# shg8/3DGS.cpp

Measured on AMD Instinct MI355X. Metric: frames/sec at 1920×1080, 1M Gaussians, higher is better.
Workload: dtype f32

## Files before the change

3dgs.cpp_amd/csrc/gs_bin_l2.hip:

```cpp
#include "gs_bin.h"

namespace gs {

struct SlabDesc {
    uint32_t off, c_total;
    uint32_t kmin;
    int32_t sh;
    uint32_t b_lo, b_hi;
    uint32_t ready;
    uint32_t pad;
    uint32_t cur[64];
};
static_assert(sizeof(SlabDesc) == 288, "descriptor layout");

struct BuildArgs {
    BinGrid g;
    uint32_t* cand;
    const uint32_t* bin_count;
    const float* depth;
    const ushort4* aabb;
    uint32_t* ranges;
    uint32_t* sorted_gid;
    Counters* counters;
    uint32_t capacity;
    uint32_t cand_capacity;
    SlabDesc* slabs;
    uint32_t slab_capacity;
    uint32_t epoch;
    uint64_t* stamps;
    const uint32_t* l1_words;
    uint32_t l1_cap;
};

__device__ __forceinline__ uint32_t bin_candidates(const BuildArgs& a, uint32_t bin) {
    return a.l1_words ? a.l1_words[(size_t)(kL1FusedCursor0 + bin) * kL1FusedStride] : a.bin_count[bin];
}
__device__ __forceinline__ uint32_t bin_offset(const BuildArgs& a, uint32_t bin) {
    return a.l1_words ? ((bin >> a.g.grid_shift) * a.g.bins_x + (bin & ((1u << a.g.grid_shift) - 1u))) * a.l1_cap : a.bin_count[kBinOffsets + bin];
}
__device__ __forceinline__ void bin_close_one_pass(const BuildArgs& a, uint32_t& c, int tid) {
    if (!a.l1_words) return;
    if (tid == 0 && c != 0) {
        atomicAdd(&a.counters->bin_entries, c);
        atomicMax(&a.counters->max_bin, c);
    }
    if (c > a.l1_cap) {
        if (tid == 0) atomicOr(&a.counters->overflow, 1u);
        c = 0;
    }
}
__device__ __forceinline__ void one_pass_visible(const BuildArgs& a) {
    if (!a.l1_words || blockIdx.x != 0 || threadIdx.x >= kVisRegions) return;
    uint32_t v = a.l1_words[(size_t)threadIdx.x * kL1FusedStride];
    for (int o = WAVE / 2; o != 0; o >>= 1) v += (uint32_t)__shfl_xor((int)v, o);
    if ((threadIdx.x & (WAVE - 1)) == 0 && v != 0) atomicAdd(&a.counters->visible, v);
}

__device__ __forceinline__ uint32_t bin_local_box(const BinGrid& g, uint32_t bin, ushort4 box) {
    const int S = 1 << g.bin_shift;
    const int ox = (int)(bin & ((1u << g.grid_shift) - 1u)) << g.bin_shift, oy = (int)(bin >> g.grid_shift) << g.bin_shift;
    const int lx0 = max((int)box.x, ox) - ox, ly0 = max((int)box.y, oy) - oy;
    const int lx1 = min((int)box.z, ox + S) - ox, ly1 = min((int)box.w, oy + S) - oy;
    return (uint32_t)lx0 | ((uint32_t)ly0 << 8) | ((uint32_t)lx1 << 16) | ((uint32_t)ly1 << 24);
}

constexpr int kBuildSlots = 16;

#ifdef GS_BUILD_TIMING
__device__ unsigned long long g_build_t[1024][10];
#define BUILD_ROW(v) uint32_t build_row = (v)
#define BUILD_ROW_SET(v) build_row = (v)
#define BUILD_T(i) do { if (threadIdx.x == 0) g_build_t[build_row][i] = wall_clock64(); } while (0)
#else
#define BUILD_ROW(v) do { } while (0)
#define BUILD_ROW_SET(v) do { } while (0)
#define BUILD_T(i) do { } while (0)
#endif

template <int R2, int THREADS, bool SORT>
struct BuildLayout {
    static constexpr int NW = THREADS / WAVE;
    static constexpr int MAXC = SORT ? THREADS * 16 : 0;
    static constexpr int SS = 64 * R2;
    static constexpr bool CACHE_BOX = SORT && R2 <= 4;
    static constexpr int TABLES = 3 * SS + kBuildSlots * SS / 2 + (SORT ? 0 : kBuildSlots * WAVE);
    static constexpr int WCNT = SORT ? NW * 256 : 0;
    static constexpr int T_OFF = (SORT && (CACHE_BOX || TABLES > MAXC)) ? 2 * MAXC : 0;
    static constexpr int WORDS = (T_OFF + TABLES > 2 * MAXC + WCNT) ? T_OFF + TABLES : 2 * MAXC + WCNT;
};

template <int R2, int THREADS, bool SORT>
__global__ __launch_bounds__(THREADS) void k_bin_build(BuildArgs a) {
    frame_stamp(a.stamps, ST_L2);
    one_pass_visible(a);
    BUILD_ROW(blockIdx.x);
    using L = BuildLayout<R2, THREADS, SORT>;
    constexpr int NW = L::NW, MAXC = L::MAXC, SS = L::SS, PER = kBuildSlots / NW;
    extern __shared__ uint32_t smem[];
    uint32_t* const s_key = smem;
    uint32_t* const s_id = smem + MAXC;
    uint32_t (*const s_wcnt)[256] = reinterpret_cast<uint32_t(*)[256]>(smem + 2 * MAXC);
    uint32_t* const t_cnt = smem + L::T_OFF;
    uint32_t* const t_cur = t_cnt + SS;
    uint16_t (*const r_cnt)[SS] = reinterpret_cast<uint16_t(*)[SS]>(t_cnt + 3 * SS);
    uint32_t* const w_ids = t_cnt + 3 * SS + kBuildSlots * SS / 2;
    __shared__ uint32_t scratch[NW];
    __shared__ uint32_t s_seg;

    const int tid = threadIdx.x, lane = tid & (WAVE - 1), w = tid / WAVE;
    const uint32_t bin = ((blockIdx.x / a.g.bins_x) << a.g.grid_shift) | (blockIdx.x % a.g.bins_x);
    BUILD_T(0);
    uint32_t c, off;
    c = bin_candidates(a, bin);
    off = bin_offset(a, bin);
    bin_close_one_pass(a, c, tid);
    if ((uint64_t)off + c > a.cand_capacity) c = 0;
    if (SORT && c > (uint32_t)MAXC) {
        if (tid == 0) atomicOr(&a.counters->overflow, 2u);
        c = 0;
    }
    BUILD_T(1);
    if (SORT && c != 0) {
        constexpr int kRounds = 16;
        {
            uint32_t g[kRounds], k[kRounds];
#pragma unroll
            for (int r = 0; r < kRounds; ++r) {
                const uint32_t e = r * THREADS + tid;
                g[r] = e < c ? a.cand[off + e] : 0u;
            }
#pragma unroll
            for (int r = 0; r < kRounds; ++r) {
                const uint32_t e = r * THREADS + tid;
                k[r] = e < c ? __float_as_uint(a.depth[g[r]]) : 0u;
            }
#pragma unroll
            for (int r = 0; r < kRounds; ++r) {
                const uint32_t e = r * THREADS + tid;
                if (e < c) {
                    s_id[e] = g[r];
                    s_key[e] = k[r];
                }
            }
        }
        BUILD_T(2);
        const uint64_t lt_mask = (1ull << lane) - 1ull;
        const int rounds = (int)((c + THREADS - 1) / THREADS);
        const uint32_t wbase = (uint32_t)w * (uint32_t)rounds * WAVE;
#pragma unroll 1
        for (int pass = 0; pass < 4; ++pass) {
            const int shift = pass * 8;
            for (int k = tid; k < NW * 256; k += THREADS) s_wcnt[k >> 8][k & 255] = 0;
            __syncthreads();
            uint32_t key[kRounds], id[kRounds], rank[kRounds];
#pragma unroll
            for (int r = 0; r < kRounds; ++r) {
                key[r] = 0;
                id[r] = 0;
                rank[r] = 0;
                if (r < rounds) {
                    const uint32_t e = wbase + r * WAVE + lane;
                    const bool ok = e < c;
                    if (ok) {
                        key[r] = s_key[e];
                        id[r] = s_id[e];
                    }
                    const uint32_t d = (key[r] >> shift) & 255u;
                    const uint64_t okm = __ballot(ok);
                    uint32_t mlo = (uint32_t)okm, mhi = (uint32_t)(okm >> 32);
#pragma unroll
                    for (int bit = 0; bit < 8; ++bit) {
                        const uint32_t mine = (d >> bit) & 1u;
                        const uint64_t b = __builtin_amdgcn_ballot_w64(mine != 0);
                        const uint32_t splat = 0u - mine;
                        mlo &= ~((uint32_t)b ^ splat);
                        mhi &= ~((uint32_t)(b >> 32) ^ splat);
                    }
                    const uint64_t m = ((uint64_t)mhi << 32) | mlo;
                    uint32_t old = 0;
                    const int leader = m ? (__ffsll((unsigned long long)m) - 1) : 0;
                    if (ok && lane == leader) {
                        old = s_wcnt[w][d];
                        s_wcnt[w][d] = old + (uint32_t)__popcll(m);
                    }
                    old = __shfl(old, leader, WAVE);
                    rank[r] = old + (uint32_t)__popcll(m & lt_mask);
                }
            }
            __syncthreads();
            {
                uint32_t cw[NW], cnt = 0;
                if (tid < 256) {
#pragma unroll
                    for (int k = 0; k < NW; ++k) {
                        cw[k] = s_wcnt[k][tid];
                        cnt += cw[k];
                    }
                }
                uint32_t all;
                uint32_t excl = block_excl_scan<THREADS>(cnt, scratch, &all);
                if (tid < 256) {
#pragma unroll
                    for (int k = 0; k < NW; ++k) {
                        s_wcnt[k][tid] = excl;
                        excl += cw[k];
                    }
                }
            }
            __syncthreads();
#pragma unroll
            for (int r = 0; r < kRounds; ++r) {
                if (r < rounds) {
                    const uint32_t e = wbase + r * WAVE + lane;
                    if (e < c) {
                        const uint32_t d = (key[r] >> shift) & 255u;
                        const uint32_t pos = s_wcnt[w][d] + rank[r];
                        s_key[pos] = key[r];
                        s_id[pos] = id[r];
                    }
                }
            }
            __syncthreads();
        }
        BUILD_T(3);
        if (L::CACHE_BOX) {
            ushort4 box[kRounds];
#pragma unroll
            for (int r = 0; r < kRounds; ++r) {
                const uint32_t e = r * THREADS + tid;
                box[r] = e < c ? a.aabb[s_id[e]] : make_ushort4(0, 0, 0, 0);
            }
#pragma unroll
            for (int r = 0; r < kRounds; ++r) {
                const uint32_t e = r * THREADS + tid;
                if (e < c) s_key[e] = bin_local_box(a.g, bin, box[r]);
            }
        }
    }
    BUILD_T(4);
    for (int t = tid; t < SS; t += THREADS) t_cnt[t] = 0;
    __syncthreads();
    const uint32_t nch = (c + WAVE - 1) / WAVE;
    auto chunk_columns = [&](uint32_t ch, uint64_t (&col)[R2], uint32_t& gid) {
        const uint32_t e = ch * WAVE + lane;
        uint32_t box = 0;
        gid = 0;
        if (e < c) {
            gid = SORT ? s_id[e] : a.cand[off + e];
            box = L::CACHE_BOX ? s_key[e] : bin_local_box(a.g, bin, a.aabb[gid]);
        }
        packed_cover_masks<R2>(a.g.bin_shift, box, col);
#pragma unroll
        for (int r = 0; r < R2; ++r)
            col[r] = (R2 == 1 || __builtin_amdgcn_ballot_w64(col[r] != 0) != 0) ? wave_transpose64(col[r], lane) : 0ull;
    };
    {
        uint32_t acc[R2];
#pragma unroll
        for (int r = 0; r < R2; ++r) acc[r] = 0;
        for (uint32_t ch = w; ch < nch; ch += NW) {
            uint64_t col[R2];
            uint32_t gid;
            chunk_columns(ch, col, gid);
#pragma unroll
            for (int r = 0; r < R2; ++r) acc[r] += (uint32_t)__popcll(col[r]);
        }
#pragma unroll
        for (int r = 0; r < R2; ++r)
            if (acc[r]) atomicAdd(&t_cnt[r * 64 + lane], acc[r]);
    }
    __syncthreads();
    BUILD_T(5);
    {
        uint32_t v[(SS + THREADS - 1) / THREADS], sum = 0;
#pragma unroll
        for (int k = 0; k < (SS + THREADS - 1) / THREADS; ++k) {
            const int t = tid * ((SS + THREADS - 1) / THREADS) + k;
            v[k] = t < SS ? t_cnt[t] : 0u;
            sum += v[k];
        }
        uint32_t d_bin;
        uint32_t excl = block_excl_scan<THREADS>(sum, scratch, &d_bin);
        if (tid == 0) {
            const uint32_t seg = d_bin ? atomicAdd(&a.counters->instances, d_bin) : 0u;
            s_seg = seg;
            if ((uint64_t)seg + d_bin > a.capacity) atomicOr(&a.counters->overflow, 1u);
        }
        __syncthreads();
        const uint32_t S = 1u << a.g.bin_shift;
        const uint32_t ox = (bin & ((1u << a.g.grid_shift) - 1u)) << a.g.bin_shift, oy = (bin >> a.g.grid_shift) << a.g.bin_shift;
#pragma unroll
        for (int k = 0; k < (SS + THREADS - 1) / THREADS; ++k) {
            const int t = tid * ((SS + THREADS - 1) / THREADS) + k;
            if (t < SS) {
                const uint32_t lx = (uint32_t)t & (S - 1), ly = (uint32_t)t >> a.g.bin_shift;
                const uint32_t x = ox + lx, y = oy + ly;
                const uint64_t start64 = (uint64_t)s_seg + excl;
                const uint32_t start = start64 > a.capacity ? a.capacity : (uint32_t)start64;
                const uint32_t end = start64 + v[k] > a.capacity ? a.capacity : (uint32_t)(start64 + v[k]);
                if (ly < S && x < a.g.tiles_x && y < a.g.tiles_y) {
                    a.ranges[2 * (y * a.g.tiles_x + x)] = v[k] ? start : 0u;
                    a.ranges[2 * (y * a.g.tiles_x + x) + 1] = v[k] ? end : 0u;
                }
                t_cur[t] = start;
            }
            excl += v[k];
        }
    }
    __syncthreads();
    BUILD_T(6);
    const __amdgpu_buffer_rsrc_t out = __builtin_amdgcn_make_buffer_rsrc(a.sorted_gid, 0, a.capacity * 4u, 0x27000);
    int par = 0;
    for (uint32_t rb = 0; rb < nch; rb += kBuildSlots, par ^= 1) {
        uint64_t col[PER][R2];
#pragma unroll
        for (int j = 0; j < PER; ++j) {
            const int slot = w * PER + j;
            uint32_t gid;
            chunk_columns(rb + slot, col[j], gid);
#pragma unroll
            for (int r = 0; r < R2; ++r) r_cnt[slot][r * 64 + lane] = (uint16_t)__popcll(col[j][r]);
            if (!SORT) w_ids[slot * WAVE + lane] = gid;
        }
        __syncthreads();
        for (int t = tid; t < SS; t += THREADS) {
            uint32_t run = 0;
#pragma unroll
            for (int k = 0; k < kBuildSlots; ++k) {
                const uint32_t v = r_cnt[k][t];
                r_cnt[k][t] = (uint16_t)run;
                run += v;
            }
            t_cur[(par ^ 1) * SS + t] = t_cur[par * SS + t] + run;
        }
        __syncthreads();
#pragma unroll
        for (int j = 0; j < PER; ++j) {
            const int slot = w * PER + j;
            const uint32_t ch = rb + slot;
            const uint32_t* ids = SORT ? s_id + (ch < nch ? ch : 0u) * WAVE : w_ids + slot * WAVE;
#pragma unroll
            for (int r = 0; r < R2; ++r) {
                if (__builtin_amdgcn_ballot_w64(col[j][r] != 0) == 0) continue;
                walk_column(col[j][r], t_cur[par * SS + r * 64 + lane] + r_cnt[slot][r * 64 + lane], out, ids);
            }
        }
    }
    BUILD_T(7);
}

#ifdef GS_BUILD_TIMING
extern "C" int gs_debug_build_timing(unsigned long long* out ) {
    return hipMemcpyFromSymbol(out, HIP_SYMBOL(g_build_t), sizeof(unsigned long long) * 1024 * 10) == hipSuccess ? 0 : -1;
}
#endif

__device__ __forceinline__ __amdgpu_buffer_rsrc_t uniform_rsrc(const void* p, uint32_t bytes) {
    const uint64_t addr = reinterpret_cast<uint64_t>(p);
    const uint32_t lo = (uint32_t)__builtin_amdgcn_readfirstlane((int)(uint32_t)addr);
    const uint32_t hi = (uint32_t)__builtin_amdgcn_readfirstlane((int)(uint32_t)(addr >> 32));
    return __builtin_amdgcn_make_buffer_rsrc(reinterpret_cast<void*>(((uint64_t)hi << 32) | lo), 0,
                                             __builtin_amdgcn_readfirstlane((int)bytes), 0x27000);
}

__device__ __forceinline__ uint32_t cover16(uint32_t pb) {
    const uint32_t lx0 = pb & 15u, ly0 = (pb >> 4) & 15u, lx1 = (pb >> 8) & 15u, ly1 = (pb >> 12) & 15u;
    const uint32_t xm = ((2u << lx1) - (1u << lx0)) & 15u;
    const uint32_t rows = (16u << (4u * ly1)) - (1u << (4u * ly0));
    return (xm * 0x1111u) & rows;
}

template <int ROUNDS>
struct FastLayout {
    static constexpr int THREADS = 1024, NW = THREADS / WAVE, MAXC = THREADS * ROUNDS;
    static constexpr int WCNT_WORDS = NW * 512 / 2;
    static constexpr int MISC_WORDS = 64 + 64 + NW * 64;
    static constexpr int TAIL = WCNT_WORDS > MISC_WORDS ? WCNT_WORDS : MISC_WORDS;
    static constexpr int WORDS = 2 * MAXC + TAIL;
};

template <int ROUNDS, int MODE = 0>
__device__ __forceinline__ void bin_fast_body(const BuildArgs& a) {
    constexpr bool SLABS = MODE != 0;
    using L = FastLayout<ROUNDS>;
    constexpr int THREADS = L::THREADS, NW = L::NW, MAXC = L::MAXC;
    extern __shared__ uint32_t smem[];
    uint32_t* const s_pay = smem;
    uint32_t* const s_key = smem + MAXC;
    uint16_t (*const s_wcnt)[512] = reinterpret_cast<uint16_t(*)[512]>(smem + 2 * MAXC);
    uint32_t* const s_id = smem + MAXC;
    uint16_t* const s_box = reinterpret_cast<uint16_t*>(smem);
    uint16_t (*const s_tbl)[64] = reinterpret_cast<uint16_t(*)[64]>(smem + MAXC / 2);
    uint32_t* const t_cnt = smem + 2 * MAXC;
    uint32_t* const t_cur = t_cnt + 64;
    uint32_t (*const s_seg)[64] = reinterpret_cast<uint32_t(*)[64]>(t_cnt + 128);
    __shared__ uint32_t scratch[NW], scratch_hi[NW];
    __shared__ uint32_t s_seg0, s_flag;
    constexpr int kSlotBits = SLABS ? 16 : 14;
    constexpr uint32_t kSlotMask = (1u << kSlotBits) - 1u;
    constexpr uint32_t kMaxInBin = SLABS ? 65535u : (uint32_t)MAXC;
    constexpr int kMaxSlabs = 16;
    __shared__ uint32_t g_cur[SLABS ? 64 : 1], t_tot[SLABS ? 64 : 1];
    __shared__ uint32_t slab_first[SLABS ? kMaxSlabs + 1 : 1];
    __shared__ uint32_t cnt2[(MODE == 1 || MODE == 3) ? kMaxSlabs : 1][64];
    __shared__ uint32_t s_fill;
    __shared__ uint16_t q_order[MODE == 3 ? 1024 : 1];
    __shared__ uint32_t q_item, q_planned;

    BUILD_ROW(MODE == 2 ? 1023u : blockIdx.x);
    if constexpr (MODE != 2) frame_stamp(a.stamps, ST_L2);
    if constexpr (MODE != 2) one_pass_visible(a);
    int tid = threadIdx.x, lane = tid & (WAVE - 1), w = tid / WAVE;
    auto screen_bin = [&](uint32_t i) { return ((i / a.g.bins_x) << a.g.grid_shift) | (i % a.g.bins_x); };
    uint32_t bin = screen_bin(MODE == 3 ? 0u : blockIdx.x);
    bool slab_item = MODE == 2;
    BUILD_T(0);
    uint32_t c_total = 0, off = 0;
    auto bin_extent = [&]() {
        c_total = (uint32_t)__builtin_amdgcn_readfirstlane((int)bin_candidates(a, bin));
        off = (uint32_t)__builtin_amdgcn_readfirstlane((int)bin_offset(a, bin));
        bin_close_one_pass(a, c_total, tid);
        if ((uint64_t)off + c_total > a.cand_capacity) c_total = 0;
        if (c_total > kMaxInBin) {
            if (tid == 0) atomicOr(&a.counters->overflow, 2u);
            c_total = 0;
        }
    };
    if constexpr (MODE == 0 || MODE == 1) bin_extent();
    if (tid == 0) s_flag = 0;
    BUILD_T(1);
#define multi (MODE == 2 ? true : (MODE == 1 ? c_total > (uint32_t)MAXC : (MODE == 3 ? (slab_item || c_total > (uint32_t)MAXC) : false)))
    uint32_t c = multi ? 0u : c_total;
    int rounds = (int)((c + THREADS - 1) / THREADS);
    typedef uint32_t u32x3 __attribute__((ext_vector_type(3)));
#define recs uniform_rsrc(a.cand + (size_t)kCandWords * off, c_total * 12u)
    uint64_t lt_mask = (1ull << lane) - 1ull;
    uint32_t wbase = (uint32_t)w * (uint32_t)rounds * WAVE;
    auto refresh = [&]() {
        int t = threadIdx.x;
        asm volatile("" : "+v"(t));
        tid = t;
        lane = t & (WAVE - 1);
        w = t / WAVE;
        lt_mask = (1ull << lane) - 1ull;
        wbase = (uint32_t)w * (uint32_t)rounds * WAVE;
    };
    auto radix_pass = [&](int shift, int db, uint32_t sub) {
        const uint32_t dmask = (1u << db) - 1u;
        for (int k = tid; k < NW * 512 / 2; k += THREADS) reinterpret_cast<uint32_t*>(&s_wcnt[0][0])[k] = 0;
        __syncthreads();
        uint32_t key[ROUNDS], pay[ROUNDS], rank[ROUNDS];
#pragma unroll
        for (int r = 0; r < ROUNDS; ++r) {
            key[r] = 0;
            pay[r] = 0;
            rank[r] = 0;
            if (r < rounds) {
                const uint32_t e = wbase + r * WAVE + lane;
                const bool ok = e < c;
                if (ok) {
                    key[r] = s_key[e] - sub;
                    pay[r] = s_pay[e];
                }
                const uint32_t d = (key[r] >> shift) & dmask;
                const uint64_t okm = __ballot(ok);
                uint32_t mlo = (uint32_t)okm, mhi = (uint32_t)(okm >> 32);
#pragma unroll
                for (int bit = 0; bit < 9; ++bit) {
                    if (bit < db) {
                        const uint32_t mine = (d >> bit) & 1u;
                        const uint64_t b = __builtin_amdgcn_ballot_w64(mine != 0);
                        const uint32_t splat = 0u - mine;
                        mlo &= ~((uint32_t)b ^ splat);
                        mhi &= ~((uint32_t)(b >> 32) ^ splat);
                    }
                }
                const uint64_t m = ((uint64_t)mhi << 32) | mlo;
                uint32_t old = 0;
                const int leader = m ? (__ffsll((unsigned long long)m) - 1) : 0;
                if (ok && lane == leader) {
                    old = s_wcnt[w][d];
                    s_wcnt[w][d] = (uint16_t)(old + (uint32_t)__popcll(m));
                }
                old = __shfl(old, leader, WAVE);
                rank[r] = old + (uint32_t)__popcll(m & lt_mask);
            }
        }
        __syncthreads();
        {
            uint32_t cw[NW], cnt = 0;
            if (tid < 512) {
#pragma unroll
                for (int k = 0; k < NW; ++k) {
                    cw[k] = s_wcnt[k][tid];
                    cnt += cw[k];
                }
            }
            uint32_t all;
            uint32_t excl = block_excl_scan<THREADS>(cnt, scratch, &all);
            if (tid < 512) {
#pragma unroll
                for (int k = 0; k < NW; ++k) {
                    s_wcnt[k][tid] = (uint16_t)excl;
                    excl += cw[k];
                }
            }
        }
        __syncthreads();
#pragma unroll
        for (int r = 0; r < ROUNDS; ++r) {
            if (r < rounds) {
                const uint32_t e = wbase + r * WAVE + lane;
                if (e < c) {
                    const uint32_t d = (key[r] >> shift) & dmask;
                    const uint32_t pos = (uint32_t)s_wcnt[w][d] + rank[r];
                    s_key[pos] = key[r];
                    s_pay[pos] = pay[r];
                }
            }
        }
        __syncthreads();
    };
    auto block_minmax = [&](uint32_t lo, uint32_t hi, uint32_t& kmin, uint32_t& span) {
#pragma unroll
        for (int d = 1; d < WAVE; d <<= 1) {
            lo = min(lo, (uint32_t)__shfl_xor((int)lo, d, WAVE));
            hi = max(hi, (uint32_t)__shfl_xor((int)hi, d, WAVE));
        }
        __syncthreads();
        if (lane == 0) {
            scratch[w] = lo;
            scratch_hi[w] = hi;
        }
        __syncthreads();
#pragma unroll
        for (int k = 0; k < NW; ++k) {
            lo = min(lo, scratch[k]);
            hi = max(hi, scratch_hi[k]);
        }
        kmin = (uint32_t)__builtin_amdgcn_readfirstlane((int)lo);
        span = (uint32_t)__builtin_amdgcn_readfirstlane((int)hi) - kmin;
    };
    auto key_range = [&](uint32_t& kmin, uint32_t& span) {
        uint32_t lo = 0xFFFFFFFFu, hi = 0u;
#pragma unroll
        for (int r = 0; r < ROUNDS; ++r) {
            const uint32_t e = r * THREADS + tid;
            if (r < rounds && e < c) {
                const uint32_t k = s_key[e];
                lo = min(lo, k);
                hi = max(hi, k);
            }
        }
        block_minmax(lo, hi, kmin, span);
    };
    auto sort_by_key_lsd = [&](uint32_t kmin, uint32_t span) {
        const int bits = span ? 32 - __builtin_clz(span) : 0;
        const int npass = (bits + 8) / 9;
        const int db = npass ? (bits + npass - 1) / npass : 0;
#pragma unroll 1
        for (int pass = 0; pass < npass; ++pass) radix_pass(pass * db, db, pass == 0 ? kmin : 0u);
        return npass ? kmin : 0u;
    };
    constexpr uint32_t kMsdBuckets = 4096, kMsdBucketMax = 64;
    uint32_t* const m_cnt = smem + 2 * MAXC;
    uint16_t* const m_start = reinterpret_cast<uint16_t*>(smem + 2 * MAXC + kMsdBuckets / 2);
    static_assert(kMsdBuckets * 4 <= L::TAIL * 4, "the bucket tables live in the counters' area");
    auto sort_by_key_msd = [&](uint32_t kmin, uint32_t span) -> bool {
        const int bits = 32 - __builtin_clz(span);
        const int sh = bits > 12 ? bits - 12 : 0;
        for (uint32_t k = tid; k < kMsdBuckets / 2; k += THREADS) m_cnt[k] = 0;
        __syncthreads();
        uint32_t key[ROUNDS], pay[ROUNDS];
#pragma unroll
        for (int r = 0; r < ROUNDS; ++r) {
            const uint32_t e = r * THREADS + tid;
            key[r] = 0;
            pay[r] = 0;
            if (r < rounds && e < c) {
                key[r] = s_key[e];
                pay[r] = s_pay[e];
                const uint32_t b = (key[r] - kmin) >> sh;
                atomicAdd(&m_cnt[b >> 1], 1u << (16u * (b & 1u)));
            }
        }
        __syncthreads();
        {
            const uint2 w2 = reinterpret_cast<const uint2*>(m_cnt)[tid];
            const uint32_t v0 = w2.x & 0xFFFFu, v1 = w2.x >> 16, v2 = w2.y & 0xFFFFu, v3 = w2.y >> 16;
            uint32_t all;
            uint32_t excl = block_excl_scan<THREADS>(v0 + v1 + v2 + v3, scratch, &all);
            if (max(max(v0, v1), max(v2, v3)) > kMsdBucketMax) s_flag = 2;
            reinterpret_cast<uint2*>(m_cnt)[tid] = make_uint2(0u, 0u);
            ushort4 st;
            st.x = (unsigned short)excl;
            st.y = (unsigned short)(excl + v0);
            st.z = (unsigned short)(excl + v0 + v1);
            st.w = (unsigned short)(excl + v0 + v1 + v2);
            reinterpret_cast<ushort4*>(m_start)[tid] = st;
        }
        __syncthreads();
        if (__builtin_amdgcn_readfirstlane((int)s_flag) == 2) {
            __syncthreads();
            if (tid == 0) s_flag = 0;
            return false;
        }
#pragma unroll
        for (int r = 0; r < ROUNDS; ++r) {
            const uint32_t e = r * THREADS + tid;
            if (r < rounds && e < c) {
                const uint32_t b = (key[r] - kmin) >> sh;
                const uint32_t old = atomicAdd(&m_cnt[b >> 1], 1u << (16u * (b & 1u)));
                const uint32_t pos = (uint32_t)m_start[b] + ((old >> (16u * (b & 1u))) & 0xFFFFu);
                s_key[pos] = key[r];
                s_pay[pos] = pay[r];
            }
        }
        __syncthreads();
        uint32_t dst[ROUNDS];
#pragma unroll
        for (int r = 0; r < ROUNDS; ++r) {
            const uint32_t e = r * THREADS + tid;
            dst[r] = 0xFFFFFFFFu;
            if (r < rounds && e < c) {
                const uint32_t k = s_key[e];
                pay[r] = s_pay[e];
                key[r] = k;
                const uint32_t b = (k - kmin) >> sh;
                const uint32_t j0 = m_start[b], j1 = b + 1 < kMsdBuckets ? (uint32_t)m_start[b + 1] : c;
                uint32_t before = 0;
                for (uint32_t j = j0; j < j1; ++j) {
                    const uint32_t kj = s_key[j];
                    before += (kj < k || (kj == k && j < e)) ? 1u : 0u;
                }
                dst[r] = j0 + before;
            }
        }
        __syncthreads();
#pragma unroll
        for (int r = 0; r < ROUNDS; ++r)
            if (dst[r] != 0xFFFFFFFFu) {
                s_key[dst[r]] = key[r];
                s_pay[dst[r]] = pay[r];
            }
        __syncthreads();
        return true;
    };
    auto sort_by_key = [&](bool try_msd) -> uint32_t {
        uint32_t kmin, span;
        key_range(kmin, span);
        if (span == 0) return 0u;
        if constexpr (ROUNDS <= 12) {
            if (try_msd && sort_by_key_msd(kmin, span)) return 0u;
        }
        return sort_by_key_lsd(kmin, span);
    };
    const int S = 1 << a.g.bin_shift;
    auto place_lists = [&](uint32_t v, uint32_t* cursors) {
        uint32_t d_bin;
        const uint32_t excl = block_excl_scan<THREADS>(v, scratch, &d_bin);
        if (tid == 0) {
            const uint32_t seg = d_bin ? atomicAdd(&a.counters->instances, d_bin) : 0u;
            s_seg0 = seg;
            if ((uint64_t)seg + d_bin > a.capacity) atomicOr(&a.counters->overflow, 1u);
        }
        __syncthreads();
        if (tid < 64) {
            const uint32_t ox = (bin & ((1u << a.g.grid_shift) - 1u)) << a.g.bin_shift, oy = (bin >> a.g.grid_shift) << a.g.bin_shift;
            const uint32_t lx = (uint32_t)tid & (uint32_t)(S - 1), ly = (uint32_t)tid >> a.g.bin_shift;
            const uint32_t x = ox + lx, y = oy + ly;
            const uint64_t start64 = (uint64_t)s_seg0 + excl;
            const uint32_t start = start64 > a.capacity ? a.capacity : (uint32_t)start64;
            const uint32_t end = start64 + v > a.capacity ? a.capacity : (uint32_t)(start64 + v);
            if (ly < (uint32_t)S && x < a.g.tiles_x && y < a.g.tiles_y) {
                a.ranges[2 * (y * a.g.tiles_x + x)] = v ? start : 0u;
                a.ranges[2 * (y * a.g.tiles_x + x) + 1] = v ? end : 0u;
            }
            cursors[tid] = start;
        }
    };
    uint32_t n_slabs = 1, g_kmin = 0;
    int g_sh = 0;
    auto plan_bin = [&]() {
    if constexpr (MODE == 1 || MODE == 3) if (!slab_item && multi) {
        uint32_t lo = 0xFFFFFFFFu, hi = 0u;
        for (uint32_t base = 0; base < c_total; base += 8 * THREADS) {
            uint32_t k[8];
#pragma unroll
            for (int r = 0; r < 8; ++r) k[r] = __builtin_amdgcn_raw_buffer_load_b32(recs, (base + r * THREADS + tid) * 12u, 0, 0);
#pragma unroll
            for (int r = 0; r < 8; ++r)
                if (base + r * THREADS + tid < c_total) {
                    lo = min(lo, k[r]);
                    hi = max(hi, k[r]);
                }
        }
        uint32_t span;
        block_minmax(lo, hi, g_kmin, span);
        const int bits = span ? 32 - __builtin_clz(span) : 0;
        g_sh = bits > 12 ? bits - 12 : 0;
        for (uint32_t k = tid; k < kMsdBuckets / 2; k += THREADS) m_cnt[k] = 0;
        for (uint32_t k = tid; k < (uint32_t)kMaxSlabs * 64u; k += THREADS) cnt2[k >> 6][k & 63u] = 0;
        __syncthreads();
        for (uint32_t base = 0; base < c_total; base += 8 * THREADS) {
            uint32_t k[8];
#pragma unroll
            for (int r = 0; r < 8; ++r) k[r] = __builtin_amdgcn_raw_buffer_load_b32(recs, (base + r * THREADS + tid) * 12u, 0, 0);
#pragma unroll
            for (int r = 0; r < 8; ++r)
                if (base + r * THREADS + tid < c_total) {
                    const uint32_t bk = (k[r] - g_kmin) >> g_sh;
                    atomicAdd(&m_cnt[bk >> 1], 1u << (16u * (bk & 1u)));
                }
        }
        __syncthreads();
        {
            const uint2 w2 = reinterpret_cast<const uint2*>(m_cnt)[tid];
            const uint32_t v0 = w2.x & 0xFFFFu, v1 = w2.x >> 16, v2 = w2.y & 0xFFFFu, v3 = w2.y >> 16;
            uint32_t all;
            const uint32_t excl = block_excl_scan<THREADS>(v0 + v1 + v2 + v3, scratch, &all);
            if (max(max(v0, v1), max(v2, v3)) > (uint32_t)MAXC) s_flag = 3;
            ushort4 st;
            st.x = (unsigned short)excl;
            st.y = (unsigned short)(excl + v0);
            st.z = (unsigned short)(excl + v0 + v1);
            st.w = (unsigned short)(excl + v0 + v1 + v2);
            reinterpret_cast<ushort4*>(m_start)[tid] = st;
            if (tid == 0) {
                slab_first[0] = 0;
                s_fill = 1;
            }
        }
        __syncthreads();
        for (int k = 0; k < kMaxSlabs; ++k) {
            const uint32_t base = m_start[slab_first[k]];
            if (c_total - base <= (uint32_t)MAXC) break;
#pragma unroll
            for (int j = 0; j < 4; ++j) {
                const uint32_t bk = 4u * tid + j;
                const uint32_t p0 = m_start[bk], p1 = bk + 1 < kMsdBuckets ? (uint32_t)m_start[bk + 1] : c_total;
                if (p0 - base <= (uint32_t)MAXC && p1 - base > (uint32_t)MAXC && bk > slab_first[k]) {
                    slab_first[k + 1] = bk;
                    s_fill = k + 2;
                }
            }
            __syncthreads();
            if (s_fill != (uint32_t)k + 2) {
                if (tid == 0) s_flag = 3;
                break;
            }
        }
        __syncthreads();
        n_slabs = (uint32_t)__builtin_amdgcn_readfirstlane((int)s_fill);
        if (tid == 0) slab_first[n_slabs] = kMsdBuckets;
        const uint32_t remaining = c_total - m_start[slab_first[n_slabs - 1]];
        if (__builtin_amdgcn_readfirstlane((int)s_flag) == 3 || remaining > (uint32_t)MAXC) {
            if (tid == 0) atomicOr(&a.counters->overflow, 2u);
            n_slabs = 0;
        }
        __syncthreads();
        if (tid == 0) s_flag = 0;
        for (uint32_t base = 0; n_slabs != 0 && base < c_total; base += 8 * THREADS) {
            uint32_t k[8], bx[8];
#pragma unroll
            for (int r = 0; r < 8; ++r) {
                const u32x3 rec = __builtin_amdgcn_raw_buffer_load_b96(recs, (base + r * THREADS + tid) * 12u, 0, 0);
                k[r] = rec.x;
                bx[r] = rec.z;
            }
#pragma unroll
            for (int r = 0; r < 8; ++r) {
                const bool valid = base + r * THREADS + tid < c_total;
                const uint32_t bk = (k[r] - g_kmin) >> g_sh;
                uint32_t sl = 0;
                for (uint32_t j = 1; j < n_slabs; ++j) sl += bk >= slab_first[j] ? 1u : 0u;
                const uint32_t pb = bx[r];
                if (S == 4) {
                    const uint32_t cm = valid ? cover16(pb) : 0u;
                    if (__builtin_amdgcn_ballot_w64(cm != 0) == 0) continue;
                    uint64_t bal[16];
#pragma unroll
                    for (int t = 0; t < 16; ++t) bal[t] = __builtin_amdgcn_ballot_w64(((cm >> t) & 1u) != 0);
                    for (uint32_t j = 0; j < n_slabs; ++j) {
                        const uint64_t mk = __builtin_amdgcn_ballot_w64(valid && sl == j);
                        if (mk == 0) continue;
                        uint32_t mine = 0;
#pragma unroll
                        for (int t = 0; t < 16; ++t) mine = lane == t ? (uint32_t)__popcll(bal[t] & mk) : mine;
                        if (lane < 16 && mine != 0) atomicAdd(&cnt2[j][lane], mine);
                    }
                } else if (valid) {
                    const uint32_t lx0 = pb & 15u, ly0 = (pb >> 4) & 15u, lx1 = (pb >> 8) & 15u, ly1 = (pb >> 12) & 15u;
                    for (uint32_t y = ly0; y <= ly1; ++y)
                        for (uint32_t x = lx0; x <= lx1; ++x) atomicAdd(&cnt2[sl][(y << a.g.bin_shift) + x], 1u);
                }
            }
        }
        __syncthreads();
        if (tid < 64) {
            uint32_t run = 0;
            for (uint32_t k = 0; k < n_slabs; ++k) {
                const uint32_t v = cnt2[k][tid];
                cnt2[k][tid] = run;
                run += v;
            }
            t_tot[tid] = run;
        }
        __syncthreads();
        place_lists(tid < 64 ? t_tot[tid] : 0u, g_cur);
        __syncthreads();
        if (tid == 0) {
            const uint32_t base = n_slabs ? atomicAdd(&a.counters->slabs, n_slabs) : 0u;
            s_seg0 = base;
            if (base + n_slabs > a.slab_capacity) atomicOr(&a.counters->overflow, 2u);
        }
        __syncthreads();
        const uint32_t dbase = (uint32_t)__builtin_amdgcn_readfirstlane((int)s_seg0);
        if (dbase + n_slabs <= a.slab_capacity) {
            auto put = [&](uint32_t* p, uint32_t v) {
                if constexpr (MODE == 3) __hip_atomic_store(p, v, __ATOMIC_RELAXED, __HIP_MEMORY_SCOPE_AGENT);
                else *p = v;
            };
            for (uint32_t k = 0; k < n_slabs; ++k) {
                SlabDesc* d = a.slabs + dbase + k;
                if (tid < 64) put(&d->cur[tid], g_cur[tid] + cnt2[k][tid]);
                if (tid == 64) {
                    put(&d->off, off);
                    put(&d->c_total, c_total);
                    put(&d->kmin, g_kmin);
                    put(reinterpret_cast<uint32_t*>(&d->sh), (uint32_t)g_sh);
                    put(&d->b_lo, slab_first[k]);
                    put(&d->b_hi, slab_first[k + 1]);
                }
            }
            if constexpr (MODE == 3) {
                asm volatile("s_waitcnt vmcnt(0)" ::: "memory");
                __syncthreads();
                if (tid == 0) {
                    for (uint32_t k = 0; k < n_slabs; ++k)
                        __hip_atomic_store(&a.slabs[dbase + k].ready, a.epoch, __ATOMIC_RELAXED, __HIP_MEMORY_SCOPE_AGENT);
                    asm volatile("s_waitcnt vmcnt(0)" ::: "memory");
                }
            }
        }
        n_slabs = 0;
    }
    };
    if constexpr (MODE == 1) plan_bin();
    auto slab_body = [&](const uint32_t slab) {
    if constexpr (SLABS) if (multi) {
        const uint32_t b_lo = slab_first[slab], b_hi = slab_first[slab + 1];
        __syncthreads();
        if (tid == 0) s_fill = 0;
        __syncthreads();
        for (uint32_t base = 0; base < c_total; base += 8 * THREADS) {
            uint32_t k[8], bx[8];
#pragma unroll
            for (int r = 0; r < 8; ++r) {
                const u32x3 rec = __builtin_amdgcn_raw_buffer_load_b96(recs, (base + r * THREADS + tid) * 12u, 0, 0);
                k[r] = rec.x;
                bx[r] = rec.z;
            }
#pragma unroll
            for (int r = 0; r < 8; ++r) {
                const uint32_t e = base + r * THREADS + tid;
                const uint32_t bk = (k[r] - g_kmin) >> g_sh;
                const bool mine = e < c_total && bk >= b_lo && bk < b_hi;
                const uint64_t mm = __builtin_amdgcn_ballot_w64(mine);
                if (mm != 0) {
                    uint32_t at = 0;
                    if (lane == __ffsll((unsigned long long)mm) - 1) at = atomicAdd(&s_fill, (uint32_t)__popcll(mm));
                    at = (uint32_t)__builtin_amdgcn_readlane((int)at, __ffsll((unsigned long long)mm) - 1) + (uint32_t)__popcll(mm & lt_mask);
                    if (mine && at < (uint32_t)MAXC) {
                        s_key[at] = k[r];
                        s_pay[at] = e | (bx[r] << kSlotBits);
                    }
                }
            }
        }
        __syncthreads();
        c = min((uint32_t)__builtin_amdgcn_readfirstlane((int)s_fill), (uint32_t)MAXC);
        rounds = (int)((c + THREADS - 1) / THREADS);
        wbase = (uint32_t)w * (uint32_t)rounds * WAVE;
    }
    for (int attempt = 0; c != 0 && attempt < 2; ++attempt) {
        uint32_t tid12 = (uint32_t)tid * 12u;
        asm volatile("" : "+v"(tid12));
        constexpr int HR = ROUNDS <= 8 ? ROUNDS : ROUNDS / 2;
        const int h_end = multi ? 0 : ROUNDS;
#pragma unroll
        for (int h = 0; h < h_end; h += HR) {
            uint32_t k[HR], b[HR];
#pragma unroll
            for (int r = 0; r < HR; ++r) {
                k[r] = 0;
                b[r] = 0;
                if (h + r < rounds) {
                    const u32x3 rec = __builtin_amdgcn_raw_buffer_load_b96(recs, tid12 + (uint32_t)(h + r) * (THREADS * 12u), 0, 0);
                    k[r] = rec.x;
                    b[r] = rec.z;
                }
            }
#pragma unroll
            for (int r = 0; r < HR; ++r) {
                const uint32_t e = (h + r) * THREADS + tid;
                if (h + r < rounds && e < c) {
                    s_key[e] = k[r];
                    s_pay[e] = e | (b[r] << kSlotBits);
                }
            }
        }
        if (attempt == 0) BUILD_T(2);
        sort_by_key(attempt == 0);
        if (attempt == 0) BUILD_T(8);
        refresh();
        uint32_t my_id[ROUNDS], run_len[(ROUNDS + 3) / 4];
        bool too_long = false;
#pragma unroll
        for (int q = 0; q < (ROUNDS + 3) / 4; ++q) run_len[q] = 0;
#pragma unroll
        for (int r = 0; r < ROUNDS; ++r) {
            const uint32_t e = r * THREADS + tid;
            my_id[r] = 0;
            if (r < rounds && e < c) {
                my_id[r] = __builtin_amdgcn_raw_buffer_load_b32(recs, (s_pay[e] & kSlotMask) * 12u + 4u, 0, 0);
                const uint32_t k = s_key[e];
                if (attempt == 0 && (e == 0 || s_key[e - 1] != k) && e + 1 < c && s_key[e + 1] == k) {
                    uint32_t more = 1;
                    while (e + more + 1 < c && more < 64 && s_key[e + more + 1] == k) ++more;
                    if (e + more + 1 < c && s_key[e + more + 1] == k) too_long = true;
                    run_len[r / 4] |= more << (8 * (r % 4));
                }
            }
        }
        if (too_long) s_flag = 1;
        __syncthreads();
        const bool redo = __builtin_amdgcn_readfirstlane((int)s_flag) != 0;
#pragma unroll
        for (int r = 0; r < ROUNDS; ++r) {
            const uint32_t e = r * THREADS + tid;
            if (r < rounds && e < c) s_id[e] = my_id[r];
        }
        __syncthreads();
        if (attempt == 0) BUILD_T(9);
        if (multi && redo) {
            if (tid == 0) atomicOr(&a.counters->overflow, 2u);
            __syncthreads();
            if (tid == 0) s_flag = 0;
            break;
        }
        if (!redo) {
#pragma unroll
            for (int r = 0; r < ROUNDS; ++r) {
                const uint32_t more = (run_len[r / 4] >> (8 * (r % 4))) & 255u;
                if (more != 0) {
                    const uint32_t e = r * THREADS + tid;
                    for (uint32_t i = e + 1; i <= e + more; ++i) {
                        const uint32_t vi = s_id[i], vp = s_pay[i];
                        uint32_t j = i;
                        while (j > e && s_id[j - 1] > vi) {
                            s_id[j] = s_id[j - 1];
                            s_pay[j] = s_pay[j - 1];
                            --j;
                        }
                        s_id[j] = vi;
                        s_pay[j] = vp;
                    }
                }
            }
            __syncthreads();
            break;
        }
        const uint32_t id_base = sort_by_key(false);
        uint32_t nk[ROUNDS], ni[ROUNDS], nb[ROUNDS];
#pragma unroll
        for (int r = 0; r < ROUNDS; ++r) {
            const uint32_t e = r * THREADS + tid;
            nk[r] = ni[r] = nb[r] = 0;
            if (r < rounds && e < c) {
                const uint32_t pw = s_pay[e];
                nk[r] = __builtin_amdgcn_raw_buffer_load_b32(recs, (pw & kSlotMask) * 12u, 0, 0);
                ni[r] = s_id[e] + id_base;
                nb[r] = pw >> kSlotBits;
            }
        }
        __syncthreads();
#pragma unroll
        for (int r = 0; r < ROUNDS; ++r) {
            const uint32_t e = r * THREADS + tid;
            if (r < rounds && e < c) {
                u32x3 rec = {nk[r], ni[r], nb[r]};
                __builtin_amdgcn_raw_buffer_store_b96(rec, recs, e * 12u, 0, 0);
            }
        }
        __threadfence_block();
        if (tid == 0) s_flag = 0;
        __syncthreads();
    }
#undef recs
    BUILD_T(3);
    refresh();
    const uint32_t nch = (c + WAVE - 1) / WAVE;
    {
        uint32_t pb16[ROUNDS];
#pragma unroll
        for (int r = 0; r < ROUNDS; ++r) {
            const uint32_t e = r * THREADS + tid;
            pb16[r] = e < c ? s_pay[e] >> kSlotBits : 0u;
        }
        __syncthreads();
        for (uint32_t k = tid; k < (uint32_t)MAXC / 2; k += THREADS) smem[MAXC / 2 + k] = 0;
        if (tid < 64) t_cnt[tid] = 0;
        __syncthreads();
#pragma unroll
        for (int r = 0; r < ROUNDS; ++r) {
            const uint32_t e = r * THREADS + tid;
            const uint32_t pb = pb16[r];
            if (e < c) s_box[e] = (uint16_t)pb;
            if (S == 4) {
                const uint32_t ch = (uint32_t)r * NW + (uint32_t)__builtin_amdgcn_readfirstlane(w);
                if (ch < nch) {
                    const uint32_t cm = e < c ? cover16(pb) : 0u;
                    uint32_t mine = 0;
#pragma unroll
                    for (int t = 0; t < 16; ++t) {
                        const uint64_t bal = __builtin_amdgcn_ballot_w64(((cm >> t) & 1u) != 0);
                        mine = lane == t ? (uint32_t)__popcll(bal) : mine;
                    }
                    s_tbl[ch][lane] = (uint16_t)mine;
                }
            }
        }
        if (S != 4) {
            __syncthreads();
            for (uint32_t ch = w; ch < nch; ch += NW) {
                const uint32_t e = ch * WAVE + lane;
                const uint32_t pb = e < c ? (uint32_t)s_box[e] : 0xFFFFu;
                uint64_t m[1];
                cover_masks<1>(3, (int)(pb & 15u), (int)((pb >> 4) & 15u), (int)((pb >> 8) & 15u) + 1, (int)(pb >> 12) + 1, m);
                if (e >= c) m[0] = 0;
                s_tbl[ch][lane] = (uint16_t)__popcll(wave_transpose64(m[0], lane));
            }
        }
    }
    __syncthreads();
    BUILD_T(4);
    {
        const int t = tid & 63, g = tid >> 6;
        const uint32_t per = (nch + NW - 1) / NW;
        const uint32_t q0 = min(nch, (uint32_t)g * per), q1 = min(nch, q0 + per);
        uint32_t sum = 0;
        for (uint32_t q = q0; q < q1; ++q) sum += s_tbl[q][t];
        s_seg[g][t] = sum;
        __syncthreads();
        if (tid < 64) {
            uint32_t run = 0;
#pragma unroll
            for (int k = 0; k < NW; ++k) {
                const uint32_t v = s_seg[k][tid];
                s_seg[k][tid] = run;
                run += v;
            }
            t_cnt[tid] = run;
        }
        __syncthreads();
        uint32_t run = s_seg[g][t];
        for (uint32_t q = q0; q < q1; ++q) {
            const uint32_t v = s_tbl[q][t];
            s_tbl[q][t] = (uint16_t)run;
            run += v;
        }
    }
    __syncthreads();
    BUILD_T(5);
    if (!multi) {
        place_lists(tid < 64 ? t_cnt[tid] : 0u, t_cur);
    } else if (tid < 64) {
        t_cur[tid] = g_cur[tid];
    }
    __syncthreads();
    BUILD_T(6);
    refresh();
    const __amdgpu_buffer_rsrc_t out = __builtin_amdgcn_make_buffer_rsrc(a.sorted_gid, 0, a.capacity * 4u, 0x27000);
    for (uint32_t ch = w; ch < nch; ch += NW) {
        const uint32_t e = ch * WAVE + lane;
        const bool valid = e < c;
        const uint32_t id = valid ? s_id[e] : 0u;
        const uint32_t pb = valid ? (uint32_t)s_box[e] : 0u;
        const int lx0 = (int)(pb & 15u), ly0 = (int)((pb >> 4) & 15u), lx1 = (int)((pb >> 8) & 15u), ly1 = (int)(pb >> 12);
        const uint32_t base = t_cur[lane] + (uint32_t)s_tbl[ch][lane];
        if (S == 4) {
            const uint32_t cm = valid ? cover16(pb) : 0u;
#pragma unroll
            for (int t = 0; t < 16; ++t) {
                const bool covered = ((cm >> t) & 1u) != 0;
                const uint64_t bal = __builtin_amdgcn_ballot_w64(covered);
                if (bal == 0) continue;
                const uint32_t rank = __builtin_amdgcn_mbcnt_hi((uint32_t)(bal >> 32), __builtin_amdgcn_mbcnt_lo((uint32_t)bal, 0u));
                const uint32_t pos = (uint32_t)__builtin_amdgcn_readlane((int)base, t) + rank;
                __builtin_amdgcn_raw_buffer_store_b32(id, out, covered ? pos * 4u : 0xFFFFFFFFu, 0, 0);
            }
        } else {
            uint64_t m[1];
            cover_masks<1>(3, lx0, ly0, lx1 + 1, ly1 + 1, m);
            if (!valid) m[0] = 0;
            walk_column(wave_transpose64(m[0], lane), base, out, s_id + ch * WAVE);
        }
    }
    if (multi && tid < 64) g_cur[tid] += t_cnt[tid];
    };
    if constexpr (MODE == 0) {
        slab_body(0u);
    } else if constexpr (MODE == 1) {
        if (n_slabs != 0) slab_body(0u);
    } else if constexpr (MODE == 3) {
        const uint32_t n_bins = a.g.bins_x * a.g.bins_y;
        {
            uint32_t* const cnt = smem;
            const uint32_t mine = (uint32_t)tid < n_bins ? bin_candidates(a, screen_bin((uint32_t)tid)) : 0u;
            cnt[tid] = mine;
            if (tid == 0) q_planned = 0;
            __syncthreads();
            if (mine > (uint32_t)MAXC) atomicAdd(&q_planned, 1u);
            if ((uint32_t)tid < n_bins) {
                uint32_t before = 0;
                for (uint32_t j = 0; j < n_bins; ++j) {
                    const uint32_t v = cnt[j];
                    before += (v > mine || (v == mine && j < (uint32_t)tid)) ? 1u : 0u;
                }
                q_order[before] = (uint16_t)tid;
            }
            __syncthreads();
        }
        const uint32_t n_planned = (uint32_t)__builtin_amdgcn_readfirstlane((int)q_planned);
        for (;;) {
            __syncthreads();
            refresh();
            if (tid == 0) {
                q_item = atomicAdd(&a.counters->q_head, 1u);
                s_flag = 0;
            }
            __syncthreads();
            const uint32_t item = (uint32_t)__builtin_amdgcn_readfirstlane((int)q_item);
            if (item < n_bins) {
                slab_item = false;
                bin = screen_bin((uint32_t)q_order[item]);
                bin_extent();
                c = multi ? 0u : c_total;
                rounds = (int)((c + THREADS - 1) / THREADS);
                wbase = (uint32_t)w * (uint32_t)rounds * WAVE;
                n_slabs = 1;
                g_kmin = 0;
                g_sh = 0;
                plan_bin();
            } else {
            const uint32_t d = item - n_bins;
            if (tid == 0) {
                uint32_t have = 0;
                if (d < a.slab_capacity) {
                    for (uint32_t spin = 0;; ++spin) {
                        if (__hip_atomic_load(&a.slabs[d].ready, __ATOMIC_RELAXED, __HIP_MEMORY_SCOPE_AGENT) == a.epoch) {
                            have = 1;
                            break;
                        }
                        if (__hip_atomic_load(&a.counters->q_bins_done, __ATOMIC_RELAXED, __HIP_MEMORY_SCOPE_AGENT) >= n_planned) {
                            asm volatile("s_waitcnt vmcnt(0)" ::: "memory");
                            have = __hip_atomic_load(&a.slabs[d].ready, __ATOMIC_RELAXED, __HIP_MEMORY_SCOPE_AGENT) == a.epoch ? 1u : 0u;
                            if (!have && d < min(__hip_atomic_load(&a.counters->slabs, __ATOMIC_RELAXED, __HIP_MEMORY_SCOPE_AGENT), a.slab_capacity) &&
                                !(__hip_atomic_load(&a.counters->overflow, __ATOMIC_RELAXED, __HIP_MEMORY_SCOPE_AGENT) & 2u))
                                atomicOr(&a.counters->overflow, 2u);
                            break;
                        }
                        if (spin > (1u << 20)) {
                            atomicOr(&a.counters->overflow, 2u);
                            break;
                        }
                        __builtin_amdgcn_s_sleep(64);
                    }
                }
                q_item = have;
            }
            __syncthreads();
            if (__builtin_amdgcn_readfirstlane((int)q_item) == 0) break;
            SlabDesc* desc = a.slabs + d;
            slab_item = true;
            auto get = [&](uint32_t* p) { return __hip_atomic_load(p, __ATOMIC_RELAXED, __HIP_MEMORY_SCOPE_AGENT); };
            off = (uint32_t)__builtin_amdgcn_readfirstlane((int)get(&desc->off));
            c_total = (uint32_t)__builtin_amdgcn_readfirstlane((int)get(&desc->c_total));
            g_kmin = (uint32_t)__builtin_amdgcn_readfirstlane((int)get(&desc->kmin));
            g_sh = __builtin_amdgcn_readfirstlane((int)get(reinterpret_cast<uint32_t*>(&desc->sh)));
            if (tid < 64) g_cur[tid] = get(&desc->cur[tid]);
            if (tid == 0) {
                slab_first[0] = get(&desc->b_lo);
                slab_first[1] = get(&desc->b_hi);
            }
            __syncthreads();
            c = 0;
            n_slabs = 1;
            }
            if (!slab_item && item < n_planned) {
                __syncthreads();
                if (tid == 0) __hip_atomic_fetch_add(&a.counters->q_bins_done, 1u, __ATOMIC_RELAXED, __HIP_MEMORY_SCOPE_AGENT);
            }
            if (n_slabs != 0) slab_body(0u);
        }
    } else {
        const uint32_t n_desc = min(a.counters->slabs, a.slab_capacity);
        for (uint32_t d = blockIdx.x; d < n_desc; d += gridDim.x) {
            const SlabDesc* desc = a.slabs + d;
            __syncthreads();
            refresh();
            off = (uint32_t)__builtin_amdgcn_readfirstlane((int)desc->off);
            c_total = (uint32_t)__builtin_amdgcn_readfirstlane((int)desc->c_total);
            g_kmin = (uint32_t)__builtin_amdgcn_readfirstlane((int)desc->kmin);
            g_sh = __builtin_amdgcn_readfirstlane(desc->sh);
            if (tid < 64) g_cur[tid] = desc->cur[tid];
            if (tid == 0) {
                slab_first[0] = desc->b_lo;
                slab_first[1] = desc->b_hi;
                s_flag = 0;
            }
            __syncthreads();
            BUILD_ROW_SET(512u + (d & 511u));
            BUILD_T(1);
            slab_body(0u);
            BUILD_T(7);
        }
        BUILD_ROW_SET(1023u);
    }
    BUILD_T(7);
}
#undef multi
template <int ROUNDS> __global__ void k_bin_fast(BuildArgs a);
template <> __global__ __launch_bounds__(1024, 4) void k_bin_fast<4>(BuildArgs a) { bin_fast_body<4>(a); }
template <> __global__ __launch_bounds__(1024, 4) void k_bin_fast<8>(BuildArgs a) { bin_fast_body<8>(a); }
template <> __global__ __launch_bounds__(1024, 4) void k_bin_fast<12>(BuildArgs a) { bin_fast_body<12>(a); }
template <> __global__ __launch_bounds__(1024, 4) void k_bin_fast<16>(BuildArgs a) { bin_fast_body<16>(a); }
constexpr int kSlabRounds = 12;
__global__ __launch_bounds__(1024, 4) void k_bin_slabs(BuildArgs a) { bin_fast_body<kSlabRounds, 1>(a); }
__global__ __launch_bounds__(1024, 4) void k_slab_work(BuildArgs a) { bin_fast_body<kSlabRounds, 2>(a); }
__global__ __launch_bounds__(1024, 4) void k_bin_queue(BuildArgs a) { bin_fast_body<kSlabRounds, 3>(a); }

template <int R2, int THREADS, bool SORT>
static hipError_t build_prepare() {
    return hipFuncSetAttribute(reinterpret_cast<const void*>(&k_bin_build<R2, THREADS, SORT>),
                               hipFuncAttributeMaxDynamicSharedMemorySize,
                               (int)(BuildLayout<R2, THREADS, SORT>::WORDS * sizeof(uint32_t)));
}
template <int ROUNDS>
static hipError_t fast_prepare() {
    return hipFuncSetAttribute(reinterpret_cast<const void*>(&k_bin_fast<ROUNDS>), hipFuncAttributeMaxDynamicSharedMemorySize,
                               (int)(FastLayout<ROUNDS>::WORDS * sizeof(uint32_t)));
}
void bin_debug_occupancy() {
    int n4 = -1, n8 = -1, n16 = -1;
    (void)hipOccupancyMaxActiveBlocksPerMultiprocessor(&n4, reinterpret_cast<const void*>(&k_bin_fast<4>), 1024,
                                                       FastLayout<4>::WORDS * sizeof(uint32_t));
    (void)hipOccupancyMaxActiveBlocksPerMultiprocessor(&n8, reinterpret_cast<const void*>(&k_bin_fast<8>), 1024,
                                                       FastLayout<8>::WORDS * sizeof(uint32_t));
    (void)hipOccupancyMaxActiveBlocksPerMultiprocessor(&n16, reinterpret_cast<const void*>(&k_bin_fast<16>), 1024,
                                                       FastLayout<16>::WORDS * sizeof(uint32_t));
    hipFuncAttributes a4{}, a8{};
    (void)hipFuncGetAttributes(&a4, reinterpret_cast<const void*>(&k_bin_fast<4>));
    (void)hipFuncGetAttributes(&a8, reinterpret_cast<const void*>(&k_bin_fast<8>));
    std::fprintf(stderr, "[occupancy] k_bin_fast<4>: %d blocks/CU (regs %d, static lds %zu, dyn %zu); <8>: %d (regs %d); <16>: %d\n", n4,
                 a4.numRegs, a4.sharedSizeBytes, FastLayout<4>::WORDS * sizeof(uint32_t), n8, a8.numRegs, n16);
}

hipError_t bin_prepare_device() {
    hipError_t e = build_prepare<4, 1024, true>();
    if (e == hipSuccess) e = build_prepare<16, 1024, true>();
    if (e == hipSuccess) e = fast_prepare<8>();
    if (e == hipSuccess) e = fast_prepare<12>();
    if (e == hipSuccess) e = fast_prepare<16>();
    if (e == hipSuccess)
        e = hipFuncSetAttribute(reinterpret_cast<const void*>(&k_bin_slabs), hipFuncAttributeMaxDynamicSharedMemorySize,
                                (int)(FastLayout<kSlabRounds>::WORDS * sizeof(uint32_t)));
    if (e == hipSuccess)
        e = hipFuncSetAttribute(reinterpret_cast<const void*>(&k_slab_work), hipFuncAttributeMaxDynamicSharedMemorySize,
                                (int)(FastLayout<kSlabRounds>::WORDS * sizeof(uint32_t)));
    if (e == hipSuccess)
        e = hipFuncSetAttribute(reinterpret_cast<const void*>(&k_bin_queue), hipFuncAttributeMaxDynamicSharedMemorySize,
                                (int)(FastLayout<kSlabRounds>::WORDS * sizeof(uint32_t)));
    return e;
}

template <int R2>
static void launch_build(const BuildArgs& a, bool sort, uint32_t bins, hipStream_t s) {
    constexpr size_t lds1 = BuildLayout<R2, 1024, true>::WORDS * sizeof(uint32_t);
    constexpr size_t lds2 = BuildLayout<R2, 1024, false>::WORDS * sizeof(uint32_t);
    if (sort) hipLaunchKernelGGL((k_bin_build<R2, 1024, true>), dim3(bins), dim3(1024), lds1, s, a);
    else hipLaunchKernelGGL((k_bin_build<R2, 1024, false>), dim3(bins), dim3(1024), lds2, s, a);
}

void launch_bin_level2(const BinLaunch& b, int level, hipStream_t s) {
    BuildArgs a;
    a.g = BinGrid{b.tiles_x, b.tiles_y, b.bins_x, b.bins_y, b.bin_shift, b.grid_shift};
    a.cand = b.cand;
    a.bin_count = b.bin_count;
    a.depth = b.depth;
    a.aabb = b.aabb;
    a.ranges = b.ranges;
    a.sorted_gid = b.sorted_gid;
    a.counters = b.counters;
    a.capacity = b.capacity;
    a.cand_capacity = b.cand_capacity;
    a.slabs = reinterpret_cast<SlabDesc*>(b.slabs);
    a.slab_capacity = b.slab_capacity;
    a.epoch = b.slab_epoch;
    a.stamps = b.stamps;
    a.l1_words = b.l1_fused_words;
    a.l1_cap = b.l1_fused_cap;
    const uint32_t bins = b.bins_x * b.bins_y;
    const bool sort = level < kBinSortLevels;
    if (sort && b.bin_shift <= 3) {
        if (level == 0) hipLaunchKernelGGL(k_bin_fast<4>, dim3(bins), dim3(1024), FastLayout<4>::WORDS * sizeof(uint32_t), s, a);
        else if (level == 1) hipLaunchKernelGGL(k_bin_fast<8>, dim3(bins), dim3(1024), FastLayout<8>::WORDS * sizeof(uint32_t), s, a);
        else if (level == 2) hipLaunchKernelGGL(k_bin_fast<12>, dim3(bins), dim3(1024), FastLayout<12>::WORDS * sizeof(uint32_t), s, a);
        else if (level == 3) hipLaunchKernelGGL(k_bin_fast<16>, dim3(bins), dim3(1024), FastLayout<16>::WORDS * sizeof(uint32_t), s, a);
        else if (b.slab_epoch != 0) {
            hipLaunchKernelGGL(k_bin_queue, dim3(bins < kQueueWorkGroups ? bins : kQueueWorkGroups), dim3(1024), FastLayout<kSlabRounds>::WORDS * sizeof(uint32_t), s, a);
        } else {
            hipLaunchKernelGGL(k_bin_slabs, dim3(bins), dim3(1024), FastLayout<kSlabRounds>::WORDS * sizeof(uint32_t), s, a);
            hipLaunchKernelGGL(k_slab_work, dim3(kSlabWorkGroups), dim3(1024), FastLayout<kSlabRounds>::WORDS * sizeof(uint32_t), s, a);
        }
    } else if (b.bin_shift <= 3) {
        launch_build<1>(a, sort, bins, s);
    } else if (b.bin_shift == 4) {
        launch_build<4>(a, sort, bins, s);
    } else {
        launch_build<16>(a, sort, bins, s);
    }
}
}
```

Baseline: 5170.

## Cut block barriers in bin build and keep transposed cover masks in registers

Several changes to the bin-build kernel. The MSD bucket-count clear now overlaps with key_range instead of taking its own barrier. place_lists uses a single-wave scan with readfirstlane in place of a block-wide exclusive scan plus __syncthreads. The 8x8 (S!=4) cover mask is computed once with a bitwise cover64 helper, and its transposed columns are kept in registers for the later walk instead of being recomputed, which also drops a pass and a barrier. Costs are extra registers (ROUNDS uint64 values per thread) that could lower occupancy, and correctness now depends on the removed zeroing of smem and t_cnt being unnecessary.

```diff
diff --git a/3dgs.cpp_amd/csrc/gs_bin_l2.hip b/3dgs.cpp_amd/csrc/gs_bin_l2.hip
--- a/3dgs.cpp_amd/csrc/gs_bin_l2.hip
+++ b/3dgs.cpp_amd/csrc/gs_bin_l2.hip
@@ -368,6 +368,14 @@
     const uint32_t xm = ((2u << lx1) - (1u << lx0)) & 15u;
     const uint32_t rows = (16u << (4u * ly1)) - (1u << (4u * ly0));
     return (xm * 0x1111u) & rows;
+}
+
+__device__ __forceinline__ uint64_t cover64(uint32_t x0, uint32_t y0, uint32_t x1, uint32_t y1) {
+    uint32_t cols = x1 > x0 ? (1u << x1) - (1u << x0) : 0u;
+    cols |= cols << 8;
+    cols |= cols << 16;
+    const uint64_t rows = y1 > y0 ? (~0ull >> (64u - 8u * (y1 - y0))) << (8u * y0) : 0ull;
+    return rows & (((uint64_t)cols << 32) | cols);
 }
 
 template <int ROUNDS>
@@ -569,8 +577,6 @@
     auto sort_by_key_msd = [&](uint32_t kmin, uint32_t span) -> bool {
         const int bits = 32 - __builtin_clz(span);
         const int sh = bits > 12 ? bits - 12 : 0;
-        for (uint32_t k = tid; k < kMsdBuckets / 2; k += THREADS) m_cnt[k] = 0;
-        __syncthreads();
         uint32_t key[ROUNDS], pay[ROUNDS];
 #pragma unroll
         for (int r = 0; r < ROUNDS; ++r) {
@@ -648,6 +654,10 @@
     };
     auto sort_by_key = [&](bool try_msd) -> uint32_t {
         uint32_t kmin, span;
+        if constexpr (ROUNDS <= 12) {
+            if (try_msd)
+                for (uint32_t k = tid; k < kMsdBuckets / 2; k += THREADS) m_cnt[k] = 0;
+        }
         key_range(kmin, span);
         if (span == 0) return 0u;
         if constexpr (ROUNDS <= 12) {
@@ -657,19 +667,19 @@
     };
     const int S = 1 << a.g.bin_shift;
     auto place_lists = [&](uint32_t v, uint32_t* cursors) {
-        uint32_t d_bin;
-        const uint32_t excl = block_excl_scan<THREADS>(v, scratch, &d_bin);
-        if (tid == 0) {
-            const uint32_t seg = d_bin ? atomicAdd(&a.counters->instances, d_bin) : 0u;
-            s_seg0 = seg;
-            if ((uint64_t)seg + d_bin > a.capacity) atomicOr(&a.counters->overflow, 1u);
-        }
-        __syncthreads();
-        if (tid < 64) {
+        if (tid < WAVE) {
+            const uint32_t incl = wave_incl_scan(v);
+            const uint32_t d_bin = (uint32_t)__builtin_amdgcn_readlane((int)incl, WAVE - 1);
+            uint32_t seg = 0;
+            if (lane == 0) {
+                seg = d_bin ? atomicAdd(&a.counters->instances, d_bin) : 0u;
+                if ((uint64_t)seg + d_bin > a.capacity) atomicOr(&a.counters->overflow, 1u);
+            }
+            seg = (uint32_t)__builtin_amdgcn_readfirstlane((int)seg);
             const uint32_t ox = (bin & ((1u << a.g.grid_shift) - 1u)) << a.g.bin_shift, oy = (bin >> a.g.grid_shift) << a.g.bin_shift;
             const uint32_t lx = (uint32_t)tid & (uint32_t)(S - 1), ly = (uint32_t)tid >> a.g.bin_shift;
             const uint32_t x = ox + lx, y = oy + ly;
-            const uint64_t start64 = (uint64_t)s_seg0 + excl;
+            const uint64_t start64 = (uint64_t)seg + (incl - v);
             const uint32_t start = start64 > a.capacity ? a.capacity : (uint32_t)start64;
             const uint32_t end = start64 + v > a.capacity ? a.capacity : (uint32_t)(start64 + v);
             if (ly < (uint32_t)S && x < a.g.tiles_x && y < a.g.tiles_y) {
@@ -1001,6 +1011,7 @@
     BUILD_T(3);
     refresh();
     const uint32_t nch = (c + WAVE - 1) / WAVE;
+    uint64_t cols[ROUNDS];
     {
         uint32_t pb16[ROUNDS];
 #pragma unroll
@@ -1009,16 +1020,14 @@
             pb16[r] = e < c ? s_pay[e] >> kSlotBits : 0u;
         }
         __syncthreads();
-        for (uint32_t k = tid; k < (uint32_t)MAXC / 2; k += THREADS) smem[MAXC / 2 + k] = 0;
-        if (tid < 64) t_cnt[tid] = 0;
-        __syncthreads();
 #pragma unroll
         for (int r = 0; r < ROUNDS; ++r) {
             const uint32_t e = r * THREADS + tid;
             const uint32_t pb = pb16[r];
-            if (e < c) s_box[e] = (uint16_t)pb;
+            const uint32_t ch = (uint32_t)r * NW + (uint32_t)__builtin_amdgcn_readfirstlane(w);
+            cols[r] = 0;
             if (S == 4) {
-                const uint32_t ch = (uint32_t)r * NW + (uint32_t)__builtin_amdgcn_readfirstlane(w);
+                if (e < c) s_box[e] = (uint16_t)pb;
                 if (ch < nch) {
                     const uint32_t cm = e < c ? cover16(pb) : 0u;
                     uint32_t mine = 0;
@@ -1029,17 +1038,10 @@
                     }
                     s_tbl[ch][lane] = (uint16_t)mine;
                 }
-            }
-        }
-        if (S != 4) {
-            __syncthreads();
-            for (uint32_t ch = w; ch < nch; ch += NW) {
-                const uint32_t e = ch * WAVE + lane;
-                const uint32_t pb = e < c ? (uint32_t)s_box[e] : 0xFFFFu;
-                uint64_t m[1];
-                cover_masks<1>(3, (int)(pb & 15u), (int)((pb >> 4) & 15u), (int)((pb >> 8) & 15u) + 1, (int)(pb >> 12) + 1, m);
-                if (e >= c) m[0] = 0;
-                s_tbl[ch][lane] = (uint16_t)__popcll(wave_transpose64(m[0], lane));
+            } else if (ch < nch) {
+                const uint64_t m = e < c ? cover64(pb & 15u, (pb >> 4) & 15u, ((pb >> 8) & 15u) + 1u, (pb >> 12) + 1u) : 0ull;
+                cols[r] = wave_transpose64(m, lane);
+                s_tbl[ch][lane] = (uint16_t)__popcll(cols[r]);
             }
         }
     }
@@ -1082,15 +1084,19 @@
     BUILD_T(6);
     refresh();
     const __amdgpu_buffer_rsrc_t out = __builtin_amdgcn_make_buffer_rsrc(a.sorted_gid, 0, a.capacity * 4u, 0x27000);
-    for (uint32_t ch = w; ch < nch; ch += NW) {
-        const uint32_t e = ch * WAVE + lane;
-        const bool valid = e < c;
-        const uint32_t id = valid ? s_id[e] : 0u;
-        const uint32_t pb = valid ? (uint32_t)s_box[e] : 0u;
-        const int lx0 = (int)(pb & 15u), ly0 = (int)((pb >> 4) & 15u), lx1 = (int)((pb >> 8) & 15u), ly1 = (int)(pb >> 12);
-        const uint32_t base = t_cur[lane] + (uint32_t)s_tbl[ch][lane];
-        if (S == 4) {
-            const uint32_t cm = valid ? cover16(pb) : 0u;
+    if (S != 4) {
+#pragma unroll
+        for (int r = 0; r < ROUNDS; ++r) {
+            const uint32_t ch = (uint32_t)r * NW + (uint32_t)__builtin_amdgcn_readfirstlane(w);
+            if (ch < nch) walk_column(cols[r], t_cur[lane] + (uint32_t)s_tbl[ch][lane], out, s_id + ch * WAVE);
+        }
+    } else {
+        for (uint32_t ch = w; ch < nch; ch += NW) {
+            const uint32_t e = ch * WAVE + lane;
+            const bool valid = e < c;
+            const uint32_t id = valid ? s_id[e] : 0u;
+            const uint32_t base = t_cur[lane] + (uint32_t)s_tbl[ch][lane];
+            const uint32_t cm = valid ? cover16((uint32_t)s_box[e]) : 0u;
 #pragma unroll
             for (int t = 0; t < 16; ++t) {
                 const bool covered = ((cm >> t) & 1u) != 0;
@@ -1100,11 +1106,6 @@
                 const uint32_t pos = (uint32_t)__builtin_amdgcn_readlane((int)base, t) + rank;
                 __builtin_amdgcn_raw_buffer_store_b32(id, out, covered ? pos * 4u : 0xFFFFFFFFu, 0, 0);
             }
-        } else {
-            uint64_t m[1];
-            cover_masks<1>(3, lx0, ly0, lx1 + 1, ly1 + 1, m);
-            if (!valid) m[0] = 0;
-            walk_column(wave_transpose64(m[0], lane), base, out, s_id + ch * WAVE);
         }
     }
     if (multi && tid < 64) g_cur[tid] += t_cnt[tid];
```

Result: no change. 5187 (median of 4 runs) (+0.3%).
